# h-walk/PySlice

Measured on AMD Instinct MI355X. Metric: slice-steps/sec (probes x frames x slices / s), potential + slice loop + exit FFT, higher is better.
Workload: dtype complex64 (f32); 1 GPU; 64-probe STEM grid, 1024x1024 grid, 200 slices, 55 MD frames per GPU (BASELINE configs[2] per-frame work), 106583 atoms, 30 mrad, 100 keV; grid=1024, slices=200, probes=64, parallelism=frames x1, world_size_checked=1, frame_slots=60, frame_batch=4

## Files before the change

### pyslice_amd/csrc/mslice.hip

```cpp
#include <hip/hip_runtime.h>

#include <algorithm>
#include <cmath>
#include <cstdarg>
#include <cstdio>
#include <cstdlib>
#include <cstring>
#include <string>
#include <vector>

#include "../../include/mslice.h"
#include "fft_generic.h"
#include "fft_pow2.h"
#include "rowtm_pass.h"
#include "potential.h"
#include "reduce.h"
#include "stream.h"
#include "tacaw_time.h"
#include "tacaw_launch.h"
#include "layer_tap.h"

using namespace msl;

namespace {
// ... 1614 lines not shown
    if (n_probes != h->cfg.n_probes) return fail(h, MSL_ERR_INVALID, "msl_set_probes: %d probes, handle has %d", n_probes, h->cfg.n_probes);
    if (mrad < 0) return fail(h, MSL_ERR_INVALID, "msl_set_probes: negative aperture");
    const msl_config& c = h->cfg;
    HIPCHK(h, hipSetDevice(c.device));
    HIPCHK(h, hipMemcpyAsync(h->d_xy, xy, 2 * sizeof(double) * n_probes, hipMemcpyHostToDevice, h->stream));
    const long long total = (long long)c.nx * c.ny * n_probes;
    const double lx = c.nx * c.dx, ly = c.ny * c.dy;
    hipLaunchKernelGGL(probe_kspace_kernel, dim3((unsigned)((total + 255) / 256)), dim3(256), 0, h->stream, h->psi0, h->d_xy,
                       n_probes, c.nx, c.ny, h->pitch, 1.0 / lx, 1.0 / ly, 1.0 / (c.nx * c.dx), 1.0 / (c.ny * c.dy),
                       (mrad * 1e-3) / c.wavelength, mrad == 0 ? 1 : 0);
    HIPCHK(h, hipGetLastError());
    int rc = fft2_inplace(h, h->psi0, n_probes, -1, 1.0f / ((float)c.nx * (float)c.ny), h->pitch);
    if (rc) return rc;
    if ((rc = transpose_probes(h))) return rc;
    HIPCHK(h, hipStreamSynchronize(h->stream));
    h->have_probes = true;
    return MSL_OK;
}

int msl_upload_probes(msl_handle* h, const float* c64, int32_t n_probes) {
    if (!h || !c64) return fail(h, MSL_ERR_INVALID, "msl_upload_probes: null argument");
    if (n_probes != h->cfg.n_probes) return fail(h, MSL_ERR_INVALID, "msl_upload_probes: %d probes, handle has %d", n_probes, h->cfg.n_probes);
    HIPCHK(h, hipSetDevice(h->cfg.device));
    HIPCHK(h, hipMemcpy2DAsync(h->psi0, (size_t)h->pitch * sizeof(float2), c64, (size_t)h->cfg.ny * sizeof(float2),
                               (size_t)h->cfg.ny * sizeof(float2), (size_t)n_probes * h->cfg.nx, hipMemcpyHostToDevice, h->stream));
    { int rc = transpose_probes(h); if (rc) return rc; }
    HIPCHK(h, hipStreamSynchronize(h->stream));
    h->have_probes = true;
    return MSL_OK;
}

static int build_potentials(msl_handle* h, const double* pos, const int32_t* Z, int64_t n, int count, int first_slot, int32_t ax1,
                            int32_t ax2, int32_t axs) {
    const msl_config& c = h->cfg;
    const size_t npix = (size_t)c.nx * c.ny;
    int z2s[104];
    for (int i = 0; i < 104; ++i) z2s[i] = -1;
    for (int64_t a = 0; a < n; ++a) {
        if (Z[a] < 1 || Z[a] > 103) return fail(h, MSL_ERR_INVALID, "msl_build_potential: atomic number %d out of 1..103", Z[a]);
        z2s[Z[a]] = 0;
    }
    int species[104], nsp = 0;
    for (int z = 1; z <= 103; ++z) if (z2s[z] == 0) { z2s[z] = nsp; species[nsp++] = z; }
    int rc;
    const bool timed = h->cfg.launch_timing != 0;
    EventPair evp_; hipEvent_t &e0 = evp_.a, &e1 = evp_.b;
    if (timed) {
        HIPCHK(h, hipEventCreate(&e0)); HIPCHK(h, hipEventCreate(&e1));
        HIPCHK(h, hipEventRecord(e0, h->stream));
    }
    if (nsp > h->ff_species_cap) {
        if ((rc = dalloc(h, &h->d_ff, npix * nsp))) return rc;
        h->ff_species_cap = nsp;
        h->ff_n = 0;
    }
    const int cx = c.nx / 2 + 1, cy = c.ny / 2 + 1;
    const size_t table_bytes_per_frame = std::max<size_t>(1, (size_t)n * (size_t)(cx + cy) * sizeof(float2));
    const int G = (int)std::max<size_t>(1, std::min<size_t>((size_t)count, (size_t)6e9 / table_bytes_per_frame));
    const int keys_per_frame = c.nz * std::max(nsp, 1);
    const int nkeys_cap = keys_per_frame * G;
    if (nkeys_cap > h->keys_cap) {
        if ((rc = dalloc(h, &h->d_counts, (size_t)nkeys_cap + 1))) return rc;
        if ((rc = dalloc(h, &h->d_start, (size_t)nkeys_cap + 1))) return rc;
        h->keys_cap = nkeys_cap;
    }
    if ((rc = ensure_atoms(h, (size_t)n * G, (size_t)n * G + (size_t)(SF_ALIGN - 1) * nkeys_cap))) return rc;
    const bool tw_axes = h->onepass && h->opx.wave2k && h->opy.wave2k && !h->V && h->transT;
    const bool t2_axes = h->onepass && h->opx.two && h->opy.two && h->opx.R == 16 && h->opy.R == 16 && !h->V;
    const bool tb_axes = h->onepass && !h->V && h->transT &&
                         (h->opx.breg || h->opx.breg2 || h->opx.cz_R) && (h->opy.breg || h->opy.breg2 || h->opy.cz_R);
    const bool herm_ifft = h->Rx && h->Ry;
    const bool herm_tb = tb_axes, herm_t2 = t2_axes, herm_tw = tw_axes;
    const bool half_rows = herm_ifft || herm_tb || herm_t2 || herm_tw;
    const float vscale = (float)(1.0 / ((double)c.nx * c.ny) / (c.dx * c.dx * c.dy * c.dy));
    struct CzRef { int R; const float2 *tw, *tw2, *bf, *bw; };
    auto cz_of = [](const msl_handle::OpDir& o) -> CzRef {
        if (o.breg2) return {64, o.tw, o.tw2, o.bf, o.bw};
        if (o.breg) return {o.R, o.tw, nullptr, o.bf, o.bw};
        return {o.cz_R, o.cz_tw, o.cz_tw2, o.cz_bf, o.cz_bw};
    };
    const bool ifft_t2 = t2_axes;
    const bool ifft_tb = h->onepass && cz_of(h->opx).R && cz_of(h->opy).R && !h->V && h->transT;
    const bool ifft_tw = tw_axes;
    bool maps_sent = false;
    for (int f0 = 0; f0 < count; f0 += G) {
        const int g = std::min(G, count - f0);
        const int slot = first_slot + f0;
        float2* const TR = h->trans + (size_t)slot * c.nz * npix;
        float2* const TRT = h->transT ? h->transT + (size_t)slot * c.nz * npix : nullptr;
        const int n_slices = c.nz * g, nkeys = keys_per_frame * g;
        const long long rows = (long long)n * g;
        bool recip_written = false;
        if (n > 0 && nsp > 0) {
            {
                msl_handle::HostStage& st = h->stage[h->stage_pos++ & 1];
                if (!st.ev) HIPCHK(h, hipEventCreateWithFlags(&st.ev, hipEventDisableTiming));
                if (st.used) HIPCHK(h, hipEventSynchronize(st.ev));
                const size_t off_sp = sizeof z2s, off_Z = (off_sp + sizeof species + 7) & ~(size_t)7;
                const size_t off_pos = (off_Z + (size_t)n * sizeof(int) + 7) & ~(size_t)7, need = off_pos + (size_t)rows * 3 * sizeof(double);
                if (need > st.bytes) {
                    if (st.buf) (void)hipHostFree(st.buf);
                    st.buf = nullptr; st.bytes = 0;
                    const size_t cap = need + need / 4;
                    if (hipHostMalloc((void**)&st.buf, cap, hipHostMallocDefault) != hipSuccess)
                        return fail(h, MSL_ERR_NOMEM, "hipHostMalloc(%zu bytes) failed", cap);
                    st.bytes = cap;
                }
                memcpy(st.buf + off_pos, pos + (size_t)f0 * n * 3, (size_t)rows * 3 * sizeof(double));
                if (!maps_sent) {
                    memcpy(st.buf, z2s, sizeof z2s);
                    memcpy(st.buf + off_sp, species, sizeof species);
                    memcpy(st.buf + off_Z, Z, (size_t)n * sizeof(int));
                    HIPCHK(h, hipMemcpyAsync(h->d_z2s, st.buf, sizeof z2s, hipMemcpyHostToDevice, h->stream));
                    HIPCHK(h, hipMemcpyAsync(h->d_species, st.buf + off_sp, nsp * sizeof(int), hipMemcpyHostToDevice, h->stream));
                    HIPCHK(h, hipMemcpyAsync(h->d_Z, st.buf + off_Z, (size_t)n * sizeof(int), hipMemcpyHostToDevice, h->stream));
                    maps_sent = true;
                }
                HIPCHK(h, hipMemcpyAsync(h->d_pos, st.buf + off_pos, (size_t)rows * 3 * sizeof(double), hipMemcpyHostToDevice, h->stream));
                HIPCHK(h, hipEventRecord(st.ev, h->stream));
                st.used = true;
            }
            HIPCHK(h, hipMemsetAsync(h->d_counts, 0, ((size_t)nkeys + 1) * sizeof(int), h->stream));
            const double lx = c.nx * c.dx, ly = c.ny * c.dy;
            if (nsp != h->ff_n || memcmp(species, h->ff_species, nsp * sizeof(int)) != 0) {
                long long tot = (long long)npix * nsp;
                hipLaunchKernelGGL(formfactor_kernel, dim3((unsigned)((tot + 255) / 256)), dim3(256), 0, h->stream, h->d_ff, h->d_abcd,
                                   h->d_species, nsp, c.nx, c.ny, 1.0 / lx, 1.0 / ly);
                memcpy(h->ff_species, species, nsp * sizeof(int));
                h->ff_n = nsp;
            }
            hipLaunchKernelGGL(atom_prep_kernel, dim3((unsigned)((rows + 255) / 256)), dim3(256), 0, h->stream, h->d_pos, h->d_Z,
                               (long long)n, g, h->d_z2s, h->d_lo, h->d_hi, c.nz, nsp, ax1, ax2, axs, 1.0 / lx, 1.0 / ly, h->d_key,
                               h->d_u1, h->d_u2, h->d_counts);
            const bool sf_stream = (double)n / std::max(1, keys_per_frame) >= 128.0 && !dbg_env("MSL_SF_TILED");
            hipLaunchKernelGGL(bin_scan_kernel, dim3(1), dim3(1024), 0, h->stream, h->d_counts, h->d_start, nkeys, sf_stream ? SF_ALIGN : 1);
            hipLaunchKernelGGL(bin_fill_kernel, dim3(nkeys), dim3(1024), 0, h->stream, h->d_key, (long long)n, keys_per_frame, h->d_start, h->d_order);
            HIPCHK(h, hipGetLastError());
            const int* n_sorted = h->d_start + nkeys;
            recip_written = true;
            const long long rows_pad = rows + (long long)(SF_ALIGN - 1) * nkeys;
            if (rows_pad > 0x7fffffffLL) return fail(h, MSL_ERR_INVALID, "msl_build_potentials: %lld padded table rows in one group exceed 2^31", rows_pad);
            const long long tx = rows_pad * cx, ty = rows_pad * cy;
            hipLaunchKernelGGL(phase_table_kernel, dim3((unsigned)((tx + 255) / 256)), dim3(256), 0, h->stream, h->d_ex, h->d_u1,
                               h->d_order, n_sorted, c.nx, cx, cx);
            hipLaunchKernelGGL(phase_table_kernel, dim3((unsigned)((ty + 255) / 256)), dim3(256), 0, h->stream, h->d_ey, h->d_u2,
                               h->d_order, n_sorted, c.ny, cy, cy);
            const bool edge_x = (c.nx % 2 == 0) && (cx % 32 == 1) && cx > 1, edge_y = (c.ny % 2 == 0) && (cy % 32 == 1) && cy > 1;
            const int tiles_x = edge_x ? cx / 32 : (cx + 31) / 32, tiles_y = edge_y ? cy / 32 : (cy + 31) / 32;
            const int n_tiles = tiles_x * tiles_y, wg_per_slice = (n_tiles + 3) / 4;
            const long long n_wg = (long long)wg_per_slice * ((n_slices + 7) / 8 * 8);
            if (n_wg > 0x7fffffffLL) return fail(h, MSL_ERR_UNSUPPORTED, "structure factor: too many workgroups");
            if (sf_stream) {
                const int n_pers = std::max(8, h->n_cus / 8 * 8);
                if (dbg_env("MSL_SF_F32"))
                    hipLaunchKernelGGL(structure_factor_stream_kernel, dim3((unsigned)n_pers), dim3(256), 0, h->stream, TR, h->d_ex, h->d_ey, h->d_ff,
                                       h->d_start, nsp, c.nx, c.ny, tiles_y, n_tiles, (int)rows_pad, half_rows ? 0 : 1, cx, cy, n_slices);
                else if ((n_tiles >= 512 || (tiles_x >= 2 && dbg_env("MSL_SF_TWO_TILES"))) && !dbg_env("MSL_SF_ONE_TILE"))
                    hipLaunchKernelGGL(structure_factor_stream_bf16x2_kernel, dim3((unsigned)n_pers), dim3(256), 4 * 128 * 64 * sizeof(float), h->stream, TR, h->d_ex, h->d_ey, h->d_ff,
                                       h->d_start, nsp, c.nx, c.ny, tiles_y, ((tiles_x + 1) / 2) * tiles_y, (int)rows_pad, half_rows ? 0 : 1, cx, cy, n_slices);
                else
                    hipLaunchKernelGGL(structure_factor_stream_bf16_kernel, dim3((unsigned)n_pers), dim3(256), 0, h->stream, TR, h->d_ex, h->d_ey, h->d_ff,
                                       h->d_start, nsp, c.nx, c.ny, tiles_y, n_tiles, (int)rows_pad, half_rows ? 0 : 1, cx, cy, n_slices);
            } else
                hipLaunchKernelGGL(structure_factor_quad_kernel, dim3((unsigned)n_wg), dim3(256), 0, h->stream, TR, h->d_ex, h->d_ey, h->d_ff,
                                   h->d_start, nsp, c.nx, c.ny, tiles_y, n_tiles, (int)rows_pad, half_rows ? 0 : 1, cx, cy, n_slices, wg_per_slice);
            if (edge_x || edge_y) {
                const int bins = (edge_x ? cy : 0) + (edge_y ? (edge_x ? cx - 1 : cx) : 0);
                for (int s0 = 0; s0 < n_slices; s0 += 65535) {
                    const int ns = std::min(65535, n_slices - s0);
                    hipLaunchKernelGGL(structure_factor_edge_kernel, dim3((bins + 127) / 128, ns), dim3(128), 0, h->stream,
                                       TR + (size_t)s0 * npix, h->d_ex, h->d_ey, h->d_ff, h->d_start + (size_t)s0 * nsp, nsp, c.nx, c.ny,
                                       edge_x ? 1 : 0, edge_y ? 1 : 0, half_rows ? 0 : 1, cx, cy);
                }
            }
            HIPCHK(h, hipGetLastError());
        }
        if (!recip_written) HIPCHK(h, hipMemsetAsync(TR, 0, npix * n_slices * sizeof(float2), h->stream));
        h->cur = nullptr;
        if (ifft_tw) {
            auto passw = [&](const msl_handle::OpDir& o, IfftTBJob j) -> int {
                constexpr int N2 = 2048;
                const size_t lds = ((size_t)N2 + 64 + (size_t)8 * (N2 + 1)) * 8;
                const long long items = (long long)(j.n_lines / 8) * j.n_images;
                const int grid = (int)std::min<long long>(items, (long long)h->n_cus);
                j.tw = o.tw; j.tw2 = o.tw2;
                (void)hipFuncSetAttribute((const void*)ifftTW_kernel, hipFuncAttributeMaxDynamicSharedMemorySize, h->lds_limit);
                hipLaunchKernelGGL(ifftTW_kernel, dim3(grid), dim3(512), lds, h->stream, j);
                HIPCHK(h, hipGetLastError());
                return mark_launch(h, K_OTHER);
            };
            IfftTBJob a{};
            a.in = TR; a.out_t = TRT; a.out_rows = nullptr;
            a.in_is = a.out_t_is = (long long)npix; a.in_pitch = c.ny; a.out_t_pitch = c.nx; a.n_lines = c.nx; a.n_line = c.ny; a.n_images = n_slices;
            a.potential = 0; a.rows_parity = -1; a.slice_mod = c.nz;
            if (herm_tw) a.n_lines = (c.nx / 2 + 1 + 7) / 8 * 8;
            if ((rc = passw(h->opy, a))) return rc;
            IfftTBJob b{};
            b.in = TRT; b.out_t = TR; b.out_rows = TRT;
            b.in_is = b.out_t_is = b.out_rows_is = (long long)npix; b.in_pitch = c.nx; b.out_t_pitch = c.ny; b.out_rows_pitch = c.nx;
            b.n_lines = c.ny; b.n_line = c.nx; b.n_images = n_slices; b.potential = 1; b.herm = herm_tw ? 1 : 0; b.slice_mod = c.nz;
            b.rows_parity = slice_is_transposed(h, 1) ? 1 : 0;
            b.scale = vscale; b.sigma_over_pi = (float)(c.sigma / M_PI);
            if ((rc = passw(h->opx, b))) return rc;
        } else if (ifft_tb) {
            auto pass = [&](const CzRef& o, IfftTBJob j) -> int {
                if (o.R == 64) {
                    constexpr int M2 = 2048, NH2 = 1024, RS = (32 * W2K_PITCH) / 2 + 1;
                    const size_t lds2 = ((size_t)M2 + 64 + NH2 + 2 + NH2 + (size_t)8 * RS) * 8;
                    const long long items2 = (long long)((j.n_lines + 7) / 8) * j.n_images;
                    const int grid2 = (int)std::min<long long>(items2, (long long)h->n_cus);
                    j.tw = o.tw; j.tw2 = o.tw2; j.bf = o.bf; j.bw = o.bw;
                    (void)hipFuncSetAttribute((const void*)ifftTB2_kernel, hipFuncAttributeMaxDynamicSharedMemorySize, h->lds_limit);
                    hipLaunchKernelGGL(ifftTB2_kernel, dim3(grid2), dim3(512), lds2, h->stream, j);
                    HIPCHK(h, hipGetLastError());
                    return mark_launch(h, K_OTHER);
                }
                const int R = o.R, M = R * R, NH = M / 2, CS = R * (R + 1) + 2;
                const size_t lds = ((size_t)M + NH + 2 + NH + (size_t)16 * CS) * 8;
                const int per_cu = std::max(1, std::min(R == 16 ? 4 : 1, (int)((size_t)h->lds_limit / lds)));
                if (R == 32 && !j.potential && !dbg_env("MSL_NO_TWO_LINE_IFFT")) {
                    constexpr int CSN = 514;
                    const size_t lds2 = ((size_t)M + NH + 2 + NH + (size_t)32 * CSN) * 8;
                    const long long items2 = (long long)((j.n_lines + 31) / 32) * j.n_images;
                    const int grid2 = (int)std::min<long long>(items2, (long long)h->n_cus);
                    j.tw = o.tw; j.bf = o.bf; j.bw = o.bw;
                    (void)hipFuncSetAttribute((const void*)ifftTB_two_kernel, hipFuncAttributeMaxDynamicSharedMemorySize, h->lds_limit);
                    hipLaunchKernelGGL(ifftTB_two_kernel, dim3(grid2), dim3(512), lds2, h->stream, j);
                    HIPCHK(h, hipGetLastError());
                    return mark_launch(h, K_OTHER);
                }
                const bool pair = R == 32 && j.herm && j.potential && !dbg_env("MSL_NO_PAIRED_IFFT");
                const long long items = (long long)((j.n_lines + (pair ? 31 : 15)) / (pair ? 32 : 16)) * j.n_images;
                const int grid = (int)std::min<long long>(items, (long long)h->n_cus * per_cu);
                j.tw = o.tw; j.bf = o.bf; j.bw = o.bw;
                if (pair) {
                    (void)hipFuncSetAttribute((const void*)ifftTB_kernel<32, true>, hipFuncAttributeMaxDynamicSharedMemorySize, h->lds_limit);
                    hipLaunchKernelGGL((ifftTB_kernel<32, true>), dim3(grid), dim3(512), lds, h->stream, j);
                } else if (R == 32) {
                    (void)hipFuncSetAttribute((const void*)ifftTB_kernel<32>, hipFuncAttributeMaxDynamicSharedMemorySize, h->lds_limit);
                    hipLaunchKernelGGL(ifftTB_kernel<32>, dim3(grid), dim3(512), lds, h->stream, j);
                } else {
                    (void)hipFuncSetAttribute((const void*)ifftTB_kernel<16>, hipFuncAttributeMaxDynamicSharedMemorySize, h->lds_limit);
                    hipLaunchKernelGGL(ifftTB_kernel<16>, dim3(grid), dim3(256), lds, h->stream, j);
                }
                HIPCHK(h, hipGetLastError());
                return mark_launch(h, K_OTHER);
            };
            IfftTBJob a{};
            a.in = TR; a.out_t = TRT; a.out_rows = nullptr;
            a.in_is = a.out_t_is = (long long)npix; a.in_pitch = c.ny; a.out_t_pitch = c.nx; a.n_lines = c.nx; a.n_line = c.ny; a.n_images = n_slices;
            a.potential = 0; a.rows_parity = -1; a.slice_mod = c.nz;
            if (herm_tb) a.n_lines = c.nx / 2 + 1;
            if ((rc = pass(cz_of(h->opy), a))) return rc;
            IfftTBJob b{};
            b.in = TRT; b.out_t = TR; b.out_rows = TRT;
            b.in_is = b.out_t_is = b.out_rows_is = (long long)npix; b.in_pitch = c.nx; b.out_t_pitch = c.ny; b.out_rows_pitch = c.nx;
            b.n_lines = c.ny; b.n_line = c.nx; b.n_images = n_slices; b.potential = 1; b.herm = herm_tb ? 1 : 0; b.slice_mod = c.nz;
            b.rows_parity = slice_is_transposed(h, 1) ? 1 : 0;
            b.scale = vscale; b.sigma_over_pi = (float)(c.sigma / M_PI);
            if ((rc = pass(cz_of(h->opx), b))) return rc;
        } else if (ifft_t2) {
            auto pass = [&](const IfftT2Job& j) -> int {
                constexpr int R = 16, N2 = R * R, N = 2 * N2;
                const size_t lds = ((size_t)2 * N2 + (size_t)16 * (N + 1)) * 8;
                const int per_cu = std::max(1, std::min(2, (int)((size_t)h->lds_limit / lds)));
                const bool pair = j.herm && j.potential && j.n_lines % 32 == 0 && !dbg_env("MSL_NO_PAIRED_IFFT");
                const long long items = (long long)(j.n_lines / (pair ? 32 : 16)) * j.n_images;
                const int grid = (int)std::min<long long>(items, (long long)h->n_cus * per_cu);
                if (pair) {
                    (void)hipFuncSetAttribute((const void*)ifftT2_kernel<16, true>, hipFuncAttributeMaxDynamicSharedMemorySize, h->lds_limit);
                    hipLaunchKernelGGL((ifftT2_kernel<16, true>), dim3(grid), dim3(256), lds, h->stream, j);
                    HIPCHK(h, hipGetLastError());
                    return mark_launch(h, K_OTHER);
                }
                (void)hipFuncSetAttribute((const void*)ifftT2_kernel<16>, hipFuncAttributeMaxDynamicSharedMemorySize, h->lds_limit);
                hipLaunchKernelGGL(ifftT2_kernel<16>, dim3(grid), dim3(256), lds, h->stream, j);
                HIPCHK(h, hipGetLastError());
                return mark_launch(h, K_OTHER);
            };
            IfftT2Job a{};
            a.in = TR; a.out_t = TRT; a.out_rows = nullptr; a.tw = h->opy.tw; a.tw2 = h->opy.tw2;
            a.in_is = a.out_t_is = (long long)npix; a.in_pitch = c.ny; a.out_t_pitch = c.nx; a.n_lines = c.nx; a.n_images = n_slices;
            a.potential = 0; a.rows_parity = -1; a.slice_mod = c.nz;
            if (herm_t2) a.n_lines = (c.nx / 2 + 1 + 15) / 16 * 16;
            if ((rc = pass(a))) return rc;
            IfftT2Job b{};
            b.in = TRT; b.out_t = TR; b.out_rows = TRT; b.tw = h->opx.tw; b.tw2 = h->opx.tw2;
            b.in_is = b.out_t_is = b.out_rows_is = (long long)npix; b.in_pitch = c.nx; b.out_t_pitch = c.ny; b.out_rows_pitch = c.nx;
            b.n_lines = c.ny; b.n_images = n_slices; b.potential = 1; b.rows_parity = 1; b.slice_mod = c.nz;
            b.herm = herm_t2 ? 1 : 0;
            b.scale = vscale; b.sigma_over_pi = (float)(c.sigma / M_PI);
            if ((rc = pass(b))) return rc;
        } else if (h->Ry) {
            RowJob r = row_job(h, TR, n_slices, c.ny);
            r.do_ifft = 1;
            if (herm_ifft) { const int Gr = 256 / h->Ry; r.nx = (c.nx / 2 + 1 + Gr - 1) / Gr * Gr; }
            if ((rc = launch_row_fast(h, r, K_OTHER))) return rc;
        } else {
            LineArgs r = row_args(h, TR, TR, n_slices, c.ny);
            r.fft1 = -1;
            if ((rc = launch_lines(h, h->plan_y, r, K_OTHER))) return rc;
        }
        if (ifft_t2 || ifft_tb || ifft_tw) {
        } else if (h->Rx) {
            ColJob k = col_job(h, TR, TR, n_slices, c.ny, c.ny);
            k.flags = COL_INV | COL_POTENTIAL; k.scale = vscale; k.sigma = (float)c.sigma; k.out_real = h->V; k.slice_mod = c.nz;
            if (h->onepass && !h->V) { k.flags |= COL_TPOT; k.tparity = h->scheme_b ? 0 : ((c.nz - 1) & 1); k.out_t = TRT; }
            if ((rc = herm_ifft ? launch_col_herm(h, k, K_OTHER) : launch_col_fast(h, k, K_OTHER))) return rc;
            if (h->onepass && h->V && (rc = transpose_odd_slices(h))) return rc;
        } else {
            LineArgs k = col_args(h, TR, TR, n_slices, c.ny, c.ny);
            k.fft1 = -1;
            k.scale = vscale;
// ... 829 lines not shown
```

### pyslice_amd/csrc/potential.h

```cpp
#pragma once
#include <hip/hip_runtime.h>
#include <stdint.h>
#include "kernel_util.h"

namespace msl {

__device__ __forceinline__ int signed_freq(int m, int n) { return (m < (n + 1) / 2) ? m : m - n; }

__global__ void formfactor_kernel(float* __restrict__ ff, const double* __restrict__ abcd,
                                  const int* __restrict__ species, int n_species, int nx, int ny,
                                  double inv_lx, double inv_ly) {
    long long i = (long long)blockIdx.x * blockDim.x + threadIdx.x;
    long long npix = (long long)nx * ny;
    if (i >= npix * n_species) return;
    int sp = (int)(i / npix);
    long long p = i - (long long)sp * npix;
    int mx = (int)(p / ny), my = (int)(p - (long long)mx * ny);
    double kx = signed_freq(mx, nx) * inv_lx, ky = signed_freq(my, ny) * inv_ly;
    double q2 = kx * kx + ky * ky;
    const double* t = abcd + (size_t)(species[sp] - 1) * 12;
    double s1 = 0.0, s2 = 0.0;
#pragma unroll
    for (int j = 0; j < 3; ++j) {
        s1 += t[j * 4 + 0] / (q2 + t[j * 4 + 1]);
// ... 353 lines not shown
        auto mma6 = [&](f32x16& acc, const sf_u32x4 (&p)[3], const sf_u32x4 (&q)[3]) {
            mma(acc, p[0], q[0]); mma(acc, p[0], q[1]); mma(acc, p[1], q[0]);
            mma(acc, p[0], q[2]); mma(acc, p[2], q[0]); mma(acc, p[1], q[1]);
        };
        auto conv = [&](sf_u32x4 (&o)[3], const float2 (&v)[8], bool imag) {
#pragma unroll
            for (int u = 0; u < 4; ++u) {
                unsigned p0, p1, p2;
                sf_split3(imag ? v[2 * u].y : v[2 * u].x, imag ? v[2 * u + 1].y : v[2 * u + 1].x, p0, p1, p2);
                o[0][u] = p0; o[1][u] = p1; o[2][u] = p2;
            }
        };
        sf_u32x4 cx[3], sx[3], cy[3], sy[3];
        auto trip = [&](int h, float2 (&x)[8], float2 (&y)[8], const float2 (&xn)[8], const float2 (&yn)[8]) {
            if (S0 + 16 * h == seg1) flush();
            mma6(A, cx, cy); conv(sy, y, true); conv(sx, x, true); __builtin_amdgcn_sched_barrier(0);
            load16(h + 2, x, y); __builtin_amdgcn_sched_barrier(0);
            mma6(C, cx, sy); conv(cx, xn, false); __builtin_amdgcn_sched_barrier(0);
            mma6(D, sx, cy); conv(cy, yn, false); __builtin_amdgcn_sched_barrier(0);
            mma6(B, sx, sy); __builtin_amdgcn_sched_barrier(0);
        };
        float2 x0[8], y0[8], x1[8], y1[8];
        if (H > 0) { load16(0, x0, y0); load16(1, x1, y1); conv(cx, x0, false); conv(cy, y0, false); }
        for (int h = 0; h < H; h += 2) {
            trip(h, x0, y0, x1, y1);
            if (h + 1 < H) trip(h + 1, x1, y1, x0, y0);
        }
        if (H > 0) flush();
        float2* out = recip + (size_t)s * nx * ny;
        const int my = ky0 + i;
        if (my > hy) continue;
#pragma unroll
        for (int r = 0; r < 16; ++r) {
            const int mx = kx0 + (r & 3) + 8 * (r >> 2) + 4 * kk;
            if (mx > hx) continue;
            store_quad_bin(out, nx, ny, mx, my, tA[r], tB[r], tC[r], tD[r], write_mx);
        }
    }
}

__global__ void __launch_bounds__(256, 1) structure_factor_stream_bf16x2_kernel(float2* __restrict__ recip, const float2* __restrict__ ex,
                                                                             const float2* __restrict__ ey, const float* __restrict__ ff,
                                                                             const int* __restrict__ start, int n_species, int nx, int ny,
                                                                             int tiles_y, int n_pairs, int n_rows, int write_mx, int px_pitch,
                                                                             int py_pitch, int n_slices) {
    extern __shared__ float sf_tot[];
    const int xcd = blockIdx.x & 7, jw = blockIdx.x >> 3, wg_x = gridDim.x >> 3;
    const int lane = threadIdx.x & 63, wave = threadIdx.x >> 6;
    const int hx = nx / 2, hy = ny / 2;
    const int i = lane & 31, kk = lane >> 5;
    const int G = (n_pairs + 3) / 4, Mx = (n_slices + 7) / 8;
    for (int q = jw; q < Mx * G; q += wg_x) {
        const int m = q / G, g = q - m * G;
        const int s = xcd + 8 * m, pair = 4 * g + wave;
        if (s >= n_slices || pair >= n_pairs) continue;
        const int kx0 = (pair / tiles_y) * 64, ky0 = (pair % tiles_y) * 32;
        const int lx0 = min(kx0 + i, hx), lx1 = min(kx0 + 32 + i, hx), ly = min(ky0 + i, hy);
        const int* st = start + s * n_species;
        const int S0 = __builtin_amdgcn_readfirstlane(st[0]), S1 = __builtin_amdgcn_readfirstlane(st[n_species]);
        const int H = (S1 - S0) >> 4;
        const unsigned rows_left = (unsigned)(n_rows - S0);
        const msl_i4v rx = make_raw_rsrc(ex + (size_t)S0 * px_pitch, (unsigned)((unsigned long long)rows_left * px_pitch * 8ull < 0xfffffff0ull ? (unsigned long long)rows_left * px_pitch * 8ull : 0xfffffff0ull));
        const msl_i4v ry = make_raw_rsrc(ey + (size_t)S0 * py_pitch, (unsigned)((unsigned long long)rows_left * py_pitch * 8ull < 0xfffffff0ull ? (unsigned long long)rows_left * py_pitch * 8ull : 0xfffffff0ull));
        const int vox0 = (8 * kk * px_pitch + lx0) * 8, vox1 = (8 * kk * px_pitch + lx1) * 8, voy = (8 * kk * py_pitch + ly) * 8;
        f32x16 A0, B0, C0, D0, A1, B1, C1, D1;
        const sf_u32x4 z4 = {0u, 0u, 0u, 0u};
        auto zero_acc = [&](f32x16& acc) { asm volatile("s_nop 15\n\ts_nop 15\n\tv_mfma_f32_32x32x16_bf16 %0, %1, %1, 0\n\ts_nop 15\n\ts_nop 15" : "=a"(acc) : "v"(z4)); };
        zero_acc(A0); zero_acc(B0); zero_acc(C0); zero_acc(D0); zero_acc(A1); zero_acc(B1); zero_acc(C1); zero_acc(D1);
        float* tot = sf_tot + (wave * 128) * 64 + lane;
#pragma unroll
        for (int r = 0; r < 128; ++r) tot[r * 64] = 0.f;
        int sp = -1, seg1 = S0;
        auto next_of = [&](int& k, int& e) { const int from = e; do { ++k; if (k >= n_species) return; e = st[k + 1]; } while (e <= from); };
        float w0[16], w1[16];
        auto load_w = [&](int spc) {
            const float* f = ff + (size_t)spc * nx * ny;
#pragma unroll
            for (int r = 0; r < 16; ++r) {
                const int row = (r & 3) + 8 * (r >> 2) + 4 * kk;
                w0[r] = f[(size_t)min(kx0 + row, hx) * ny + ly];
                w1[r] = f[(size_t)min(kx0 + 32 + row, hx) * ny + ly];
            }
        };
#pragma unroll
        for (int r = 0; r < 16; ++r) { w0[r] = 0.f; w1[r] = 0.f; }
        next_of(sp, seg1);
        if (sp < n_species) load_w(sp);
        auto flush = [&]() {
            asm volatile("s_nop 15\n\ts_nop 15\n\ts_nop 15\n\ts_nop 15\n\ts_nop 15\n\ts_nop 15" ::: "memory");
#pragma unroll
            for (int r = 0; r < 16; ++r) {
                float* t = tot + r * 64;
                t[0 * 1024] = fmaf(w0[r], A0[r], t[0 * 1024]); t[1 * 1024] = fmaf(w0[r], B0[r], t[1 * 1024]);
                t[2 * 1024] = fmaf(w0[r], C0[r], t[2 * 1024]); t[3 * 1024] = fmaf(w0[r], D0[r], t[3 * 1024]);
                t[4 * 1024] = fmaf(w1[r], A1[r], t[4 * 1024]); t[5 * 1024] = fmaf(w1[r], B1[r], t[5 * 1024]);
                t[6 * 1024] = fmaf(w1[r], C1[r], t[6 * 1024]); t[7 * 1024] = fmaf(w1[r], D1[r], t[7 * 1024]);
            }
            zero_acc(A0); zero_acc(B0); zero_acc(C0); zero_acc(D0); zero_acc(A1); zero_acc(B1); zero_acc(C1); zero_acc(D1);
            next_of(sp, seg1);
            if (sp < n_species) load_w(sp);
        };
        auto load16 = [&](int h, float2 (&xa)[8], float2 (&xb)[8], float2 (&y)[8]) {
            const int r0 = __builtin_amdgcn_readfirstlane(16 * h);
#pragma unroll
            for (int u = 0; u < 8; ++u) {
                const msl_f2v a = msl_raw_buffer_load_f2(rx, vox0, (r0 + u) * px_pitch * 8, 0);
                const msl_f2v c = msl_raw_buffer_load_f2(rx, vox1, (r0 + u) * px_pitch * 8, 0);
                const msl_f2v b = msl_raw_buffer_load_f2(ry, voy, (r0 + u) * py_pitch * 8, 0);
                xa[u] = make_float2(a.x, a.y); xb[u] = make_float2(c.x, c.y); y[u] = make_float2(b.x, b.y);
            }
        };
        auto mma = [&](f32x16& acc, const sf_u32x4& a, const sf_u32x4& b) { asm volatile("v_mfma_f32_32x32x16_bf16 %0, %1, %2, %0" : "+a"(acc) : "v"(a), "v"(b)); };
        auto mma6 = [&](f32x16& acc, const sf_u32x4 (&p)[3], const sf_u32x4 (&qq)[3]) {
            mma(acc, p[0], qq[0]); mma(acc, p[0], qq[1]); mma(acc, p[1], qq[0]);
            mma(acc, p[0], qq[2]); mma(acc, p[2], qq[0]); mma(acc, p[1], qq[1]);
        };
        auto conv = [&](sf_u32x4 (&o)[3], const float2 (&v)[8], bool imag) {
#pragma unroll
            for (int u = 0; u < 4; ++u) {
                unsigned p0, p1, p2;
                sf_split3(imag ? v[2 * u].y : v[2 * u].x, imag ? v[2 * u + 1].y : v[2 * u + 1].x, p0, p1, p2);
                o[0][u] = p0; o[1][u] = p1; o[2][u] = p2;
            }
        };
        sf_u32x4 cx0[3], sx0[3], cx1[3], sx1[3], cy[3], sy[3];
        auto trip = [&](int h, float2 (&xa)[8], float2 (&xb)[8], float2 (&y)[8], const float2 (&xan)[8], const float2 (&xbn)[8], const float2 (&yn)[8]) {
            if (S0 + 16 * h == seg1) flush();
            mma6(A0, cx0, cy); mma6(A1, cx1, cy); conv(sy, y, true); conv(sx0, xa, true); conv(sx1, xb, true); __builtin_amdgcn_sched_barrier(0);
            load16(h + 2, xa, xb, y); __builtin_amdgcn_sched_barrier(0);
            mma6(C0, cx0, sy); mma6(C1, cx1, sy); conv(cx0, xan, false); conv(cx1, xbn, false); __builtin_amdgcn_sched_barrier(0);
            mma6(D0, sx0, cy); mma6(D1, sx1, cy); conv(cy, yn, false); __builtin_amdgcn_sched_barrier(0);
            mma6(B0, sx0, sy); mma6(B1, sx1, sy); __builtin_amdgcn_sched_barrier(0);
        };
        float2 xa0[8], xb0[8], y0[8], xa1[8], xb1[8], y1[8];
        if (H > 0) { load16(0, xa0, xb0, y0); load16(1, xa1, xb1, y1); conv(cx0, xa0, false); conv(cx1, xb0, false); conv(cy, y0, false); }
        for (int h = 0; h < H; h += 2) {
            trip(h, xa0, xb0, y0, xa1, xb1, y1);
            if (h + 1 < H) trip(h + 1, xa1, xb1, y1, xa0, xb0, y0);
        }
        if (H > 0) flush();
        float2* out = recip + (size_t)s * nx * ny;
        const int my = ky0 + i;
        if (my > hy) continue;
#pragma unroll
        for (int r = 0; r < 16; ++r) {
            const int mx = kx0 + (r & 3) + 8 * (r >> 2) + 4 * kk;
            const float* t = tot + r * 64;
            if (mx <= hx) store_quad_bin(out, nx, ny, mx, my, t[0 * 1024], t[1 * 1024], t[2 * 1024], t[3 * 1024], write_mx);
            if (mx + 32 <= hx) store_quad_bin(out, nx, ny, mx + 32, my, t[4 * 1024], t[5 * 1024], t[6 * 1024], t[7 * 1024], write_mx);
        }
    }
}


__global__ void __launch_bounds__(128) structure_factor_edge_kernel(float2* __restrict__ recip, const float2* __restrict__ ex,
                                                                    const float2* __restrict__ ey, const float* __restrict__ ff,
                                                                    const int* __restrict__ start, int n_species, int nx, int ny,
                                                                    int edge_x, int edge_y, int write_mx, int px_pitch, int py_pitch) {
    const int s = blockIdx.y;
    const int hx = nx / 2, hy = ny / 2;
    const int n_row = edge_x ? hy + 1 : 0;
    const int n_col = edge_y ? (edge_x ? hx : hx + 1) : 0;
    const int i = blockIdx.x * blockDim.x + threadIdx.x;
    if (i >= n_row + n_col) return;
    const int mx = i < n_row ? hx : i - n_row, my = i < n_row ? i : hy;
    float tA = 0.f, tB = 0.f, tC = 0.f, tD = 0.f;
    for (int sp = 0; sp < n_species; ++sp) {
        const int a0 = start[s * n_species + sp], a1 = start[s * n_species + sp + 1];
        float A = 0.f, B = 0.f, C = 0.f, D = 0.f;
        int a = a0;
        for (; a + 8 <= a1; a += 8) {
            float2 x[8], y[8];
#pragma unroll
            for (int u = 0; u < 8; ++u) { x[u] = ex[(size_t)(a + u) * px_pitch + mx]; y[u] = ey[(size_t)(a + u) * py_pitch + my]; }
#pragma unroll
            for (int u = 0; u < 8; ++u) {
                A = fmaf(x[u].x, y[u].x, A); B = fmaf(x[u].y, y[u].y, B); C = fmaf(x[u].x, y[u].y, C); D = fmaf(x[u].y, y[u].x, D);
            }
        }
        for (; a < a1; ++a) {
            const float2 x = ex[(size_t)a * px_pitch + mx], y = ey[(size_t)a * py_pitch + my];
            A = fmaf(x.x, y.x, A); B = fmaf(x.y, y.y, B); C = fmaf(x.x, y.y, C); D = fmaf(x.y, y.x, D);
        }
        const float w = ff[(size_t)sp * nx * ny + (size_t)mx * ny + my];
        tA = fmaf(w, A, tA); tB = fmaf(w, B, tB); tC = fmaf(w, C, tC); tD = fmaf(w, D, tD);
    }
    store_quad_bin(recip + (size_t)s * nx * ny, nx, ny, mx, my, tA, tB, tC, tD, write_mx);
}

__global__ void probe_kspace_kernel(float2* __restrict__ psik, const double* __restrict__ xy, int P, int nx, int ny,
                                    int pitch, double inv_lx, double inv_ly, double kfreq_x, double kfreq_y, double radius,
                                    int plane_wave) {
    long long i = (long long)blockIdx.x * blockDim.x + threadIdx.x;
    long long npix = (long long)nx * ny;
    if (i >= npix * P) return;
    int p = (int)(i / npix);
    long long q = i - (long long)p * npix;
    int mx = (int)(q / ny), my = (int)(q - (long long)mx * ny);
    const long long o = ((long long)p * nx + mx) * pitch + my;
    if (plane_wave) {
        psik[o] = (mx == 0 && my == 0) ? make_float2((float)npix, 0.f) : make_float2(0.f, 0.f);
        return;
    }
    int fx = signed_freq(mx, nx), fy = signed_freq(my, ny);
    double kx = fx * kfreq_x, ky = fy * kfreq_y;
    bool inside = sqrt(kx * kx + ky * ky) < radius;
    if (!inside) { psik[o] = make_float2(0.f, 0.f); return; }
    double t = fx * ((double)(nx / 2) / nx + xy[2 * p] * inv_lx) + fy * ((double)(ny / 2) / ny + xy[2 * p + 1] * inv_ly);
    t -= rint(t);
    float sn, cs;
    sincospif((float)(2.0 * t), &sn, &cs);
    psik[o] = make_float2(cs, sn);
}

__global__ void probe_ramp_kernel(float2* __restrict__ out, const float2* __restrict__ basek,
                                  const double* __restrict__ xy, int P, int nx, int ny, int pitch, double inv_lx, double inv_ly) {
    long long i = (long long)blockIdx.x * blockDim.x + threadIdx.x;
    long long npix = (long long)nx * ny;
    if (i >= npix * P) return;
    int p = (int)(i / npix);
    long long q = i - (long long)p * npix;
    int mx = (int)(q / ny), my = (int)(q - (long long)mx * ny);
    const long long o = ((long long)p * nx + mx) * pitch + my;
    double t = signed_freq(mx, nx) * (xy[2 * p] * inv_lx) + signed_freq(my, ny) * (xy[2 * p + 1] * inv_ly);
    t -= rint(t);
    float sn, cs;
    sincospif((float)(2.0 * t), &sn, &cs);
    float2 b = basek[q];
    out[o] = make_float2(b.x * cs - b.y * sn, b.x * sn + b.y * cs);
}

__global__ void transmission_kernel(float2* __restrict__ t, const float* __restrict__ V, long long n, float sigma) {
    long long i = (long long)blockIdx.x * blockDim.x + threadIdx.x;
    if (i >= n) return;
    float sn, cs;
    sincosf(sigma * V[i], &sn, &cs);
    t[i] = make_float2(cs, sn);
}

}
```

Baseline: 239,800 slice-steps/s.

## Add LDS-panel MFMA structure factor kernel covering 64x64 output blocks

Adds a structure-factor kernel where four waves jointly stage x and y phase-table panels, split into three bf16 terms, into double-buffered LDS. Each wave then computes one 32x32 tile of a 64x64 block with bf16 MFMAs, so panel loads are shared across tiles instead of being fetched per tile. Global loads for later chunks are software-pipelined and interleaved with the MFMAs using scheduling barriers. The new kernel becomes the default path when its LDS size fits the device limit, and the two-tile kernel now runs only when requested by environment flag. The cost is a __syncthreads per chunk and one workgroup per CU because of the launch bounds.

```diff
diff --git a/pyslice_amd/csrc/mslice.hip b/pyslice_amd/csrc/mslice.hip
--- a/pyslice_amd/csrc/mslice.hip
+++ b/pyslice_amd/csrc/mslice.hip
@@ -1790,13 +1790,19 @@
             if (n_wg > 0x7fffffffLL) return fail(h, MSL_ERR_UNSUPPORTED, "structure factor: too many workgroups");
             if (sf_stream) {
                 const int n_pers = std::max(8, h->n_cus / 8 * 8);
+                const size_t x2_lds = 4 * 128 * 64 * sizeof(float);
                 if (dbg_env("MSL_SF_F32"))
                     hipLaunchKernelGGL(structure_factor_stream_kernel, dim3((unsigned)n_pers), dim3(256), 0, h->stream, TR, h->d_ex, h->d_ey, h->d_ff,
                                        h->d_start, nsp, c.nx, c.ny, tiles_y, n_tiles, (int)rows_pad, half_rows ? 0 : 1, cx, cy, n_slices);
-                else if ((n_tiles >= 512 || (tiles_x >= 2 && dbg_env("MSL_SF_TWO_TILES"))) && !dbg_env("MSL_SF_ONE_TILE"))
-                    hipLaunchKernelGGL(structure_factor_stream_bf16x2_kernel, dim3((unsigned)n_pers), dim3(256), 4 * 128 * 64 * sizeof(float), h->stream, TR, h->d_ex, h->d_ey, h->d_ff,
+                else if (!dbg_env("MSL_SF_ONE_TILE") && !dbg_env("MSL_SF_TWO_TILES") && SF_PANEL_LDS_BYTES <= h->lds_limit) {
+                    (void)hipFuncSetAttribute((const void*)structure_factor_panel_kernel, hipFuncAttributeMaxDynamicSharedMemorySize, SF_PANEL_LDS_BYTES);
+                    hipLaunchKernelGGL(structure_factor_panel_kernel, dim3((unsigned)n_pers), dim3(256), SF_PANEL_LDS_BYTES, h->stream, TR, h->d_ex, h->d_ey, h->d_ff,
+                                       h->d_start, nsp, c.nx, c.ny, tiles_x, tiles_y, half_rows ? 0 : 1, cx, cy, n_slices);
+                } else if (tiles_x >= 2 && dbg_env("MSL_SF_TWO_TILES") && !dbg_env("MSL_SF_ONE_TILE") && x2_lds <= (size_t)h->lds_limit) {
+                    (void)hipFuncSetAttribute((const void*)structure_factor_stream_bf16x2_kernel, hipFuncAttributeMaxDynamicSharedMemorySize, (int)x2_lds);
+                    hipLaunchKernelGGL(structure_factor_stream_bf16x2_kernel, dim3((unsigned)n_pers), dim3(256), x2_lds, h->stream, TR, h->d_ex, h->d_ey, h->d_ff,
                                        h->d_start, nsp, c.nx, c.ny, tiles_y, ((tiles_x + 1) / 2) * tiles_y, (int)rows_pad, half_rows ? 0 : 1, cx, cy, n_slices);
-                else
+                } else
                     hipLaunchKernelGGL(structure_factor_stream_bf16_kernel, dim3((unsigned)n_pers), dim3(256), 0, h->stream, TR, h->d_ex, h->d_ey, h->d_ff,
                                        h->d_start, nsp, c.nx, c.ny, tiles_y, n_tiles, (int)rows_pad, half_rows ? 0 : 1, cx, cy, n_slices);
             } else
diff --git a/pyslice_amd/csrc/potential.h b/pyslice_amd/csrc/potential.h
--- a/pyslice_amd/csrc/potential.h
+++ b/pyslice_amd/csrc/potential.h
@@ -529,6 +529,145 @@
     }
 }
 
+#define SF_PANEL_ENTRIES (2 * 2 * 3 * 2 * 64)
+#define SF_PANEL_LDS_BYTES (2 * SF_PANEL_ENTRIES * 16)
+typedef __bf16 sf_bf16x8 __attribute__((ext_vector_type(8)));
+__global__ void __launch_bounds__(256, 1) structure_factor_panel_kernel(float2* __restrict__ recip, const float2* __restrict__ ex,
+                                                                     const float2* __restrict__ ey, const float* __restrict__ ff,
+                                                                     const int* __restrict__ start, int n_species, int nx, int ny,
+                                                                     int tiles_x, int tiles_y, int write_mx, int px_pitch, int py_pitch,
+                                                                     int n_slices) {
+    extern __shared__ sf_u32x4 sf_panel[];
+    const int xcd = blockIdx.x & 7, jw = blockIdx.x >> 3, wg_x = gridDim.x >> 3;
+    const int lane = threadIdx.x & 63, wave = __builtin_amdgcn_readfirstlane(threadIdx.x >> 6);
+    const int hx = nx / 2, hy = ny / 2;
+    const int i = lane & 31, kk = lane >> 5;
+    const int mty = (tiles_y + 1) / 2, G = ((tiles_x + 1) / 2) * mty, Mx = (n_slices + 7) / 8;
+    const int ld_p = wave >> 1, ld_kk = wave & 1;
+    const float2* const tab = ld_p ? ey : ex;
+    const int pitch = ld_p ? py_pitch : px_pitch, hmax = ld_p ? hy : hx;
+    const int tx = wave & 1, ty = wave >> 1;
+    for (int q = jw; q < Mx * G; q += wg_x) {
+        const int m = q / G, g = q - m * G;
+        const int s = xcd + 8 * m;
+        if (s >= n_slices) continue;
+        const int gx = g / mty, gy = g - gx * mty;
+        const int kx0 = 64 * gx + 32 * tx, ky0 = 64 * gy + 32 * ty;
+        const int ly = min(ky0 + i, hy);
+        const int col = min(64 * (ld_p ? gy : gx) + lane, hmax);
+        const int* st = start + s * n_species;
+        const int S0 = __builtin_amdgcn_readfirstlane(st[0]), S1 = __builtin_amdgcn_readfirstlane(st[n_species]);
+        const int H = (S1 - S0) >> 4;
+        auto load = [&](int j, float2 (&r)[8]) {
+            const msl_i4v rs = make_raw_rsrc(tab + ((long long)S0 + 16LL * j) * pitch, j < H ? 16u * (unsigned)pitch * 8u : 0u);
+            const int vo = (8 * ld_kk * pitch + col) * 8;
+#pragma unroll
+            for (int u = 0; u < 8; ++u) {
+                const msl_f2v a = msl_raw_buffer_load_f2(rs, vo, u * pitch * 8, 0);
+                r[u] = make_float2(a.x, a.y);
+            }
+        };
+        auto split_store = [&](int b, const float2 (&r)[8]) {
+            sf_u32x4* p = sf_panel + b * SF_PANEL_ENTRIES + (ld_p * 12 + ld_kk) * 64 + lane;
+#pragma unroll
+            for (int c = 0; c < 2; ++c) {
+                sf_u32x4 o[3];
+#pragma unroll
+                for (int u = 0; u < 4; ++u) {
+                    unsigned p0, p1, p2;
+                    sf_split3(c ? r[2 * u].y : r[2 * u].x, c ? r[2 * u + 1].y : r[2 * u + 1].x, p0, p1, p2);
+                    o[0][u] = p0; o[1][u] = p1; o[2][u] = p2;
+                }
+#pragma unroll
+                for (int k = 0; k < 3; ++k) p[((c * 3 + k) * 2) * 64] = o[k];
+            }
+        };
+        auto operand = [&](int b, int panel, int c, int k, int t) -> sf_u32x4 {
+            return sf_panel[b * SF_PANEL_ENTRIES + (((panel * 2 + c) * 3 + k) * 2 + kk) * 64 + 32 * t + i];
+        };
+        f32x16 tA = {0}, tB = {0}, tC = {0}, tD = {0};
+        f32x16 A = {0}, B = {0}, C = {0}, D = {0};
+        int sp = -1, seg1 = S0, spn = -1, segn1 = S0;
+        auto next_of = [&](int& k, int& e) { const int from = e; do { ++k; if (k >= n_species) return; e = st[k + 1]; } while (e <= from); };
+        float wc[16], wn[16];
+        auto load_w = [&](int spc, float (&w)[16]) {
+            const float* f = ff + (size_t)spc * nx * ny;
+#pragma unroll
+            for (int r = 0; r < 16; ++r) w[r] = f[(size_t)min(kx0 + (r & 3) + 8 * (r >> 2) + 4 * kk, hx) * ny + ly];
+        };
+#pragma unroll
+        for (int r = 0; r < 16; ++r) { wc[r] = 0.f; wn[r] = 0.f; }
+        next_of(sp, seg1);
+        spn = sp; segn1 = seg1;
+        if (sp < n_species) { load_w(sp, wc); next_of(spn, segn1); if (spn < n_species) load_w(spn, wn); }
+        auto flush = [&]() {
+#pragma unroll
+            for (int r = 0; r < 16; ++r) {
+                tA[r] = fmaf(wc[r], A[r], tA[r]); tB[r] = fmaf(wc[r], B[r], tB[r]);
+                tC[r] = fmaf(wc[r], C[r], tC[r]); tD[r] = fmaf(wc[r], D[r], tD[r]);
+                A[r] = 0.f; B[r] = 0.f; C[r] = 0.f; D[r] = 0.f;
+                wc[r] = wn[r];
+            }
+            sp = spn; seg1 = segn1;
+            if (sp < n_species) { next_of(spn, segn1); if (spn < n_species) load_w(spn, wn); }
+        };
+        auto mma = [](const f32x16& acc, const sf_u32x4& a, const sf_u32x4& b) {
+            return __builtin_amdgcn_mfma_f32_32x32x16_bf16(__builtin_bit_cast(sf_bf16x8, a), __builtin_bit_cast(sf_bf16x8, b), acc, 0, 0, 0);
+        };
+        auto trip = [&](int h, float2 (&r)[8]) {
+            const int b = h & 1;
+            sf_u32x4 cx[3], sx[3], cy[3], sy[3];
+#pragma unroll
+            for (int k = 0; k < 3; ++k) {
+                cx[k] = operand(b, 0, 0, k, tx); sx[k] = operand(b, 0, 1, k, tx);
+                cy[k] = operand(b, 1, 0, k, ty); sy[k] = operand(b, 1, 1, k, ty);
+            }
+            split_store(b ^ 1, r);
+            load(h + 3, r);
+            constexpr int P[6] = {0, 0, 1, 0, 2, 1}, Q[6] = {0, 1, 0, 2, 0, 1};
+#pragma unroll
+            for (int t = 0; t < 6; ++t) {
+                A = mma(A, cx[P[t]], cy[Q[t]]);
+                C = mma(C, cx[P[t]], sy[Q[t]]);
+                D = mma(D, sx[P[t]], cy[Q[t]]);
+                B = mma(B, sx[P[t]], sy[Q[t]]);
+            }
+            __builtin_amdgcn_sched_group_barrier(0x100, 12, 0);
+            __builtin_amdgcn_sched_group_barrier(0x002, 8, 0);
+#pragma unroll
+            for (int t = 0; t < 24; ++t) {
+                __builtin_amdgcn_sched_group_barrier(0x008, 1, 0);
+                __builtin_amdgcn_sched_group_barrier(0x002, 4, 0);
+            }
+            __syncthreads();
+        };
+        float2 r0[8], r1[8];
+        if (H > 0) {
+            load(0, r0); load(1, r1);
+            split_store(0, r0);
+            load(2, r0);
+            __syncthreads();
+        }
+        for (int h = 0; sp < n_species;) {
+            const int h1 = (seg1 - S0) >> 4;
+            if (h < h1 && (h & 1)) { trip(h, r0); ++h; }
+            for (; h + 1 < h1; h += 2) { trip(h, r1); trip(h + 1, r0); }
+            if (h < h1) { trip(h, r1); ++h; }
+            flush();
+        }
+        if (kx0 >= 32 * tiles_x || ky0 >= 32 * tiles_y) continue;
+        float2* out = recip + (size_t)s * nx * ny;
+        const int my = ky0 + i;
+        if (my > hy) continue;
+#pragma unroll
+        for (int r = 0; r < 16; ++r) {
+            const int mx = kx0 + (r & 3) + 8 * (r >> 2) + 4 * kk;
+            if (mx > hx) continue;
+            store_quad_bin(out, nx, ny, mx, my, tA[r], tB[r], tC[r], tD[r], write_mx);
+        }
+    }
+}
+
 
 __global__ void __launch_bounds__(128) structure_factor_edge_kernel(float2* __restrict__ recip, const float2* __restrict__ ex,
                                                                     const float2* __restrict__ ey, const float* __restrict__ ff,
```

Measured after the change: 240,600 slice-steps/s, median of 6. No clear change (+0.3%).
